# mathworks/turtle_kv

Measured on AMD Instinct MI355X. Metric: filter-build Mkeys/s (device-resident), 16B keys @10 bits/key; bit-exact, higher is better.
Workload: dtype u64; 1 GPU; Bloom @10 bits/key: 100000000 x 16B keys per GPU, 16384-key leaves (6104 filters on rank 0); keys_per_gpu=100000000, total_keys=100000000, key_bytes=16, leaf_keys=16384, bits_per_key=10, filter=bloom-blocked512, parallelism=leaf-sharded x1

## Files before the change

### turtle_kv_amd/_build.py

```python
from __future__ import annotations

import fcntl
import hashlib
import os
import subprocess

HERE = os.path.dirname(os.path.abspath(__file__))
ROOT = os.path.dirname(HERE)
LIB = os.path.join(HERE, "libtkv_amq.so")
SOURCES = [os.path.join(HERE, "csrc", "tkv_amq_kernels.hip"),
           os.path.join(HERE, "csrc", "tkv_amq_open_scan.hip"),
           os.path.join(HERE, "csrc", "tkv_amq_find.hip"),
           os.path.join(HERE, "csrc", "tkv_amq_walk.hip"),
           os.path.join(HERE, "csrc", "tkv_amq_stage.cpp")]
DEPS = SOURCES + [os.path.join(HERE, "csrc", "tkv_amq_device.h"),
                  os.path.join(HERE, "csrc", "tkv_amq_verify.h"),
                  os.path.join(ROOT, "include", "tkv_amq.h")]
HIPCC = os.environ.get("HIPCC", "/opt/rocm/bin/hipcc")
FLAGS = ["-O3", "--offload-arch=gfx950", "-std=c++17", "-shared", "-fPIC",
         "-Wall", "-Wno-unused-function", "-I" + os.path.join(ROOT, "include")]


STAMP = LIB + ".src"
LOCK = LIB + ".lock"


def source_digest() -> str:
    h = hashlib.sha256(" ".join([HIPCC, *FLAGS]).encode())
    for d in DEPS:
        with open(d, "rb") as f:
            h.update(f.read())
    return h.hexdigest()


def stale() -> bool:
    if not (os.path.exists(LIB) and os.path.exists(STAMP)):
        return True
    with open(STAMP) as f:
        return f.read().strip() != source_digest()


def build(force: bool = False) -> str:
    if not force and not stale():
        return LIB
    with open(LOCK, "a") as lk:
        fcntl.flock(lk, fcntl.LOCK_EX)
        try:
            if force or stale():
# ... 18 lines not shown
```

### turtle_kv_amd/csrc/tkv_amq_kernels.hip

```cpp
#include <hip/hip_runtime.h>

#include <algorithm>
#include <mutex>
#include <type_traits>
#include <vector>

#include <math.h>
#include <stdint.h>
#include <string.h>
#include <stdlib.h>

#include "tkv_amq.h"
#include "tkv_amq_device.h"

#if defined(TKV_DIAG_RING) && !defined(TKV_AMQ_EXPERIMENT_BUILD)
#error "TKV_DIAG_RING is a diagnostic: build it only as an experiment library (-DTKV_AMQ_EXPERIMENT_BUILD)"
#endif

namespace tkv {

struct BloomSeeds {
  uint64_t seed[kMaxBloomHashes];
  uint64_t rhinit16[kMaxBloomHashes];
  uint64_t seed_p5[kMaxBloomHashes];
};

constexpr BloomSeeds make_bloom_seeds()
{
  BloomSeeds t{};
  for (uint32_t i = 0; i < kMaxBloomHashes; ++i) {
    t.seed[i] = bloom_seed(i);
    t.rhinit16[i] = xxh16_rhinit(t.seed[i]);
    t.seed_p5[i] = t.seed[i] + kP5;
  }
  return t;
}

__constant__ BloomSeeds c_bloom = make_bloom_seeds();

enum KeyMode : int { kKey16 = 0, kKeyFixed = 1, kKeyVar = 2, kKey24 = 3, kKeyLoc = 4 };

typedef uint32_t u32x4_t __attribute__((ext_vector_type(4)));

__device__ inline uint4 load_nt16(const void* p)
{
  const u32x4_t v = __builtin_nontemporal_load(static_cast<const u32x4_t*>(p));
// ... 94 lines not shown
TKV_INLINE auto with_bloom_key_at(const uint8_t* keys, const uint64_t* offs, uint32_t stride, uint64_t i, F&& f)
{
  uint32_t len;
  const uint8_t* p = key_at<MODE>(keys, offs, stride, i, len);
  if (len < 32) return f(BloomShort(p, len));
  return f(BloomLong{p, len});
}

__device__ inline void lds_barrier()
{
  asm volatile("s_waitcnt lgkmcnt(0)\n\ts_barrier" ::: "memory");
}

__device__ inline void lds_set_bit(uint32_t* blk, uint32_t bit)
{
  uint32_t word;
  asm("v_bfe_u32 %0, %1, 5, 4" : "=v"(word) : "v"(bit));
  atomicOr(blk + word, 1u << (bit & 31));
}

TKV_INLINE void global_set_bit(uint32_t* blk, uint32_t bit)
{
  bit &= kBloomBitMask;
  atomicOr(blk + (bit >> 5), 1u << (bit & 31));
}

typedef __attribute__((address_space(3))) uint32_t lds_u32_t;
__device__ inline uint32_t lds_addr(const void* p)
{
  return (uint32_t)reinterpret_cast<uintptr_t>(p);
}
TKV_INLINE uint32_t* lds_ptr(uint32_t a) { return (uint32_t*)reinterpret_cast<lds_u32_t*>((uintptr_t)a); }

template <int K, bool kMask = false, typename H>
TKV_INLINE void bloom_insert(uint32_t* s_bits, uint32_t nb, uint32_t k, const H& x, uint32_t first = 0)
{
  const uint64_t h0 = x.h0();
  uint32_t block = (uint32_t)bloom_block(h0, nb);
  asm("" : "+v"(block));
  uint32_t* blk = lds_ptr((block << 6) + (lds_addr(s_bits) - (first << 6)));
  lds_set_bit(blk, (uint32_t)h0);
  bloom_ladder<K>(x, k, [&](uint32_t, uint32_t b) { lds_set_bit(blk, kMask ? b & kBloomBitMask : b); });
}

template <int K, int MODE>
__device__ inline void bloom_insert_any(uint32_t* s_bits, uint32_t nb, uint32_t k,
                                        const uint8_t* p, uint32_t len)
{
  if (len < 32) bloom_insert<K>(s_bits, nb, k, BloomShort(p, len));
  else bloom_insert<0, true>(s_bits, nb, k, BloomLong{p, len});
}

__device__ inline void write_bloom_header(uint8_t* payload, const tkv_amq_segment& sg, int part)
{
  uint64_t w0, w1;
  const uint64_t nb = sg.n_blocks;
  switch (part) {
    case 0: w0 = kBloomMagic; w1 = 512ull * nb; break;
    case 1: w0 = sg.src_page_id; w1 = 0; break;
    case 2: w0 = 8ull * nb; w1 = nb | ((uint64_t)sg.hash_count << 32) | (2ull << 48); break;
    default: w0 = sg.n_keys; w1 = 0; break;
  }
  ulonglong2 v;
  v.x = w0;
  v.y = w1;
  reinterpret_cast<ulonglong2*>(payload)[part] = v;
}

constexpr uint64_t kLayoutVqf = 0x746c69665f667176ull;
constexpr uint64_t kLayoutBloom = 0x746c666d6f6f6c62ull;

__device__ inline void write_page_header(uint8_t* out, const tkv_amq_segment& sg, uint64_t layout,
                                         uint32_t part)
{
  if (!(sg.page_flags & TKV_AMQ_PAGE_IMAGE)) return;
  uint8_t* page = out + sg.out_offset - kPackedPageHeaderBytes;
  const uint32_t size = 1u << ((sg.page_flags >> 8) & 31u);
  uint4 v = {0, 0, 0, 0};
  if (part == 1) {
    v.x = (uint32_t)layout;
    v.y = (uint32_t)(layout >> 32);
    v.w = (uint32_t)kPackedPageHeaderBytes + sg.payload_bytes;
  } else if (part == 2) {
// ... 7 lines not shown
TKV_INLINE uint64_t sgpr_addr(const uint8_t* base)
{
  uint64_t a = reinterpret_cast<uint64_t>(base);
  asm("" : "+s"(a));
  return a;
}

template <typename T>
TKV_INLINE T load_sbase(uint64_t sbase, uint32_t lane_off, uint32_t imm = 0)
{
  return *reinterpret_cast<const __attribute__((address_space(1))) T*>(sbase + lane_off + imm);
}

template <int K, uint32_t NT = 256>
__device__ inline void bloom_keys16_lds(const uint4* __restrict__ kp, uint32_t n, uint32_t nb,
                                        uint32_t k, uint32_t* s_bits)
{
  const uint32_t tid = threadIdx.x;
  constexpr int U = 4;
  constexpr uint32_t C = NT * U;
  const uint8_t* cb = reinterpret_cast<const uint8_t*>(kp);
  uint32_t lane_off = tid * 16;
  uint32_t base = 0;
  for (; n - base >= C; base += C, cb += C * 16) {
    asm volatile("" : "+v"(lane_off));
    uint4 kv[U];
#pragma unroll
    for (int u = 0; u < U; ++u) {
      const u32x4_t v = load_sbase<u32x4_t>(sgpr_addr(cb + u * NT * 16), lane_off);
      kv[u] = uint4{v.x, v.y, v.z, v.w};
    }
#pragma unroll
    for (int u = 0; u < U; ++u) {
      bloom_insert<K>(s_bits, nb, k, Bloom16(kv[u]));
      __builtin_amdgcn_sched_barrier(0);
    }
  }
  if (base < n) {
    uint4 kv[U];
#pragma unroll
    for (int u = 0; u < U; ++u) {
      const uint32_t i = base + u * NT + tid;
      if (i < n) kv[u] = kp[i];
    }
#pragma unroll
    for (int u = 0; u < U; ++u) {
      const uint32_t i = base + u * NT + tid;
      if (i < n) bloom_insert<K>(s_bits, nb, k, Bloom16(kv[u]));
    }
  }
}

template <int K, int L, uint32_t NT>
__device__ inline void bloom_keysL_lds(const uint64_t* __restrict__ kp, uint32_t n, uint32_t nb,
                                       uint32_t k, uint32_t* s_bits)
{
  constexpr int N = L / 8;
  const uint32_t tid = threadIdx.x;
  constexpr int U = 2;
  constexpr uint32_t C = NT * U;
  const uint8_t* cb = reinterpret_cast<const uint8_t*>(kp);
  uint32_t lane_off = tid * L;
  uint32_t base = 0;
  for (; n - base >= C; base += C, cb += C * L) {
    asm volatile("" : "+v"(lane_off));
    uint64_t lanes[U][N];
#pragma unroll
    for (int u = 0; u < U; ++u) {
      const uint64_t sb = sgpr_addr(cb + u * NT * L);
#pragma unroll
      for (int w = 0; w < N; ++w) lanes[u][w] = load_sbase<uint64_t>(sb, lane_off, w * 8);
    }
#pragma unroll
    for (int u = 0; u < U; ++u) {
      bloom_insert<K>(s_bits, nb, k, BloomFixed<L>(lanes[u]));
      __builtin_amdgcn_sched_barrier(0);
    }
  }
  if (base < n) {
    uint64_t lanes[U][N];
#pragma unroll
    for (int u = 0; u < U; ++u) {
      const uint32_t i = min(base + u * NT + tid, n - 1);
#pragma unroll
      for (int w = 0; w < N; ++w) lanes[u][w] = kp[(uint64_t)i * N + w];
    }
#pragma unroll
    for (int u = 0; u < U; ++u) {
      if (base + u * NT + tid < n) {
        bloom_insert<K>(s_bits, nb, k, BloomFixed<L>(lanes[u]));
      }
    }
  }
}

template <int MODE, uint32_t NT>
__device__ inline void bloom_leaf_image(const uint8_t* __restrict__ keys,
                                        const uint64_t* __restrict__ offs, uint32_t stride,
                                        const tkv_amq_segment& sg, uint32_t kb, uint32_t ke,
                                        uint32_t* s_bits)
{
  const uint32_t n = ke - kb, nb = sg.n_blocks, k = sg.hash_count;
  if constexpr (MODE == kKey16) {
    const uint4* kp = reinterpret_cast<const uint4*>(keys) + sg.key_begin + kb;
    if (k == 7) bloom_keys16_lds<7, NT>(kp, n, nb, k, s_bits);
    else if (k == 8) bloom_keys16_lds<8, NT>(kp, n, nb, k, s_bits);
    else bloom_keys16_lds<0, NT>(kp, n, nb, k, s_bits);
  } else if constexpr (MODE == kKey24) {
    const uint64_t* kp = reinterpret_cast<const uint64_t*>(keys) + 3 * (sg.key_begin + kb);
    if (n != 0) {
      if (k == 7) bloom_keysL_lds<7, 24, NT>(kp, n, nb, k, s_bits);
      else if (k == 8) bloom_keysL_lds<8, 24, NT>(kp, n, nb, k, s_bits);
      else bloom_keysL_lds<0, 24, NT>(kp, n, nb, k, s_bits);
    }
  } else {
    for (uint32_t i = kb + threadIdx.x; i < ke; i += NT) {
      uint32_t len;
      const uint8_t* p = key_at<MODE>(keys, offs, stride, sg.key_begin + i, len);
      if (k == 7) bloom_insert_any<7, MODE>(s_bits, nb, k, p, len);
      else if (k == 8) bloom_insert_any<8, MODE>(s_bits, nb, k, p, len);
      else bloom_insert_any<0, MODE>(s_bits, nb, k, p, len);
    }
  }
// ... 74 lines not shown
  const bool sh = len < 32;
  const uint32_t n8 = len >> 3, nb = len & 3;
  uint64_t l[3];
#pragma unroll
  for (uint32_t j = 0; j < 3; ++j) l[j] = ld64_unaligned(sh && j < n8 ? p + 8 * j : safe);
  const uint8_t* q = p + 8 * n8;
  const uint32_t t4 = ld32_unaligned(sh && (len & 4) ? q : safe);
  q += len & 4;
  const uint32_t c0 = *(sh && nb > 0 ? q : safe), c1 = *(sh && nb > 1 ? q + 1 : safe),
                 c2 = *(sh && nb > 2 ? q + 2 : safe);
  const uint32_t tb = c0 | c1 << 8 | c2 << 16;
  const uint32_t tlo = (len & 4) ? t4 : tb;
  w.a = u32x4_b{lo32(l[0]), hi32(l[0]), lo32(l[1]), hi32(l[1])};
  w.b = u32x4_b{lo32(l[2]), hi32(l[2]), tlo, tb};
  if (n8 == 0) { w.a.x = tlo; w.a.y = tb; }
  else if (n8 == 1) { w.a.z = tlo; w.a.w = tb; }
  else if (n8 == 2) { w.b.x = tlo; w.b.y = tb; }
  w.d = 0;
}

struct VarKey {
  KeyWin w;
  uint32_t len;
  const uint8_t* p;
};

template <int K>
__device__ inline void var_key_insert(uint32_t* s_bits, uint32_t nb, uint32_t k, const VarKey& v)
{
  if (v.len < 32) {
    uint64_t l[3];
    uint32_t t4, tb;
    key_win_parts(v.w, v.len, l, t4, tb);
    bloom_insert<K>(s_bits, nb, k, BloomShort(v.len, l, t4, tb));
  } else {
    bloom_insert_any<K, kKeyVar>(s_bits, nb, k, v.p, v.len);
  }
}

template <uint32_t NT, int K>
__device__ void bloom_var_sorted_image(const uint8_t* __restrict__ keys, const uint64_t* __restrict__ offs,
                                       const tkv_amq_segment& sg, uint32_t kb, uint32_t ke,
                                       uint32_t* s_bits, uint32_t* s_aux, uint64_t key_end)
{
  constexpr uint32_t C = kVarChunk<NT>, U = C / NT;
  uint32_t* bins = s_aux;
  uint32_t* start = s_aux + kVarBins;
  uint2* kl = reinterpret_cast<uint2*>(s_aux + 2 * kVarBins);
  const uint32_t tid = threadIdx.x, nb = sg.n_blocks, k = sg.hash_count;
  const uint64_t* o = offs + sg.key_begin;
  const uint8_t* safe = reinterpret_cast<const uint8_t*>(offs);
  for (uint32_t c0 = kb; c0 < ke; c0 += C) {
    const uint32_t cn = min(C, ke - c0);
    const uint64_t base = o[c0];
    if (tid < kVarBins) bins[tid] = 0;
    __syncthreads();
    uint32_t bin[U], rank[U], rel[U], len[U];
#pragma unroll
    for (uint32_t u = 0; u < U; ++u) {
      const uint32_t j = u * NT + tid;
      const uint32_t i = c0 + min(j, cn - 1);
      const uint64_t b = o[i];
      const uint64_t l = o[i + 1] - b;
      rel[u] = (uint32_t)(b - base);
      len[u] = (uint32_t)l;
      bin[u] = l < 32 ? (uint32_t)l : 32u;
      rank[u] = j < cn ? atomicAdd(bins + bin[u], 1u) : 0u;
// ... 15 lines not shown
      const uint32_t j = u * NT + tid;
      if (j < cn) kl[start[bin[u]] + rank[u]] = make_uint2(rel[u], len[u]);
    }
    __syncthreads();
    const uint8_t* kbase = keys + base;
    const VarRsrc vr = var_rsrc(keys, base, o[c0 + cn], key_end);
    VarKey A, B;
    auto load = [&](uint32_t q, VarKey& v) {
      const uint2 e = kl[min(q, cn - 1)];
      if (vr.nrec) key_win_load(vr, e.x, v.w);
      else key_win_load_clamped(kbase + e.x, e.y, safe, v.w);
      v.len = e.y;
      v.p = kbase + e.x;
    };
    load(tid, A);
    for (uint32_t q = tid; q < cn; q += 2 * NT) {
      load(q + NT, B);
      var_key_insert<K>(s_bits, nb, k, A);
      if (q + NT >= cn) break;
      load(q + 2 * NT, A);
      var_key_insert<K>(s_bits, nb, k, B);
    }
    __syncthreads();
  }
}

template <int MODE, uint32_t NT>
__global__ __launch_bounds__(NT) void bloom_build_lds(const uint8_t* __restrict__ keys,
                                                       const uint64_t* __restrict__ offs,
                                                       uint32_t stride,
                                                       const tkv_amq_segment* __restrict__ segs,
                                                       uint8_t* __restrict__ out, uint32_t var_sort)
{
  extern __shared__ uint32_t s_lds[];
  const bool sorted = MODE == kKeyVar && var_sort;
  uint32_t* s_bits = s_lds + (sorted ? kVarAuxWords<NT> : 0u);
  const tkv_amq_segment sg = segs[blockIdx.x];
  const uint32_t n = sg.n_keys, nb = sg.n_blocks, k = sg.hash_count;
  if (k == 0) return;
  const uint32_t tid = threadIdx.x;
  const uint32_t nwords = nb * 16;

  for (uint32_t w = tid; w < nwords; w += NT) s_bits[w] = 0;
  __syncthreads();
  if constexpr (MODE == kKeyVar) {
    if (sorted) {
      const tkv_amq_segment& last = segs[gridDim.x - 1];
      const uint64_t key_end = offs[last.key_begin + last.n_keys];
      if (k == 7) bloom_var_sorted_image<NT, 7>(keys, offs, sg, 0, n, s_bits, s_lds, key_end);
      else if (k == 8) bloom_var_sorted_image<NT, 8>(keys, offs, sg, 0, n, s_bits, s_lds, key_end);
      else bloom_var_sorted_image<NT, 0>(keys, offs, sg, 0, n, s_bits, s_lds, key_end);
    } else {
      bloom_leaf_image<MODE, NT>(keys, offs, stride, sg, 0, n, s_bits);
    }
  } else {
    bloom_leaf_image<MODE, NT>(keys, offs, stride, sg, 0, n, s_bits);
  }
  __syncthreads();

  uint8_t* payload = out + sg.out_offset;
  if (tid < 4) write_bloom_header(payload, sg, tid);
  else if (tid < 8) write_page_header(out, sg, kLayoutBloom, tid - 4);
  uint4* dst = reinterpret_cast<uint4*>(payload + kBloomHeader);
  const uint4* src = reinterpret_cast<const uint4*>(s_bits);
  for (uint32_t q = tid; q < nb * 4; q += NT) dst[q] = src[q];
}

constexpr uint32_t kSplitThreads = 512;
constexpr uint32_t kSplitMaxParts = 16;
constexpr uint32_t kMergeThreads = 256;

template <int MODE>
__global__ __launch_bounds__(kSplitThreads) void bloom_build_split(
    const uint8_t* __restrict__ keys, const uint64_t* __restrict__ offs, uint32_t stride,
    const tkv_amq_segment* __restrict__ segs, uint32_t parts, uint8_t* __restrict__ ws,
    uint64_t img_stride)
{
  constexpr uint32_t NT = kSplitThreads;
  extern __shared__ uint32_t s_bits[];
  const uint32_t seg = blockIdx.x / parts, part = blockIdx.x - seg * parts;
  const tkv_amq_segment sg = segs[seg];
  const uint32_t n = sg.n_keys, nb = sg.n_blocks;
  if (sg.hash_count == 0) return;
  const uint32_t tid = threadIdx.x;
  for (uint32_t w = tid; w < nb * 16; w += NT) s_bits[w] = 0;
  __syncthreads();
  const uint32_t chunk = (n + parts - 1) / parts;
  const uint32_t kb = min(n, part * chunk), ke = min(n, kb + chunk);
  bloom_leaf_image<MODE, NT>(keys, offs, stride, sg, kb, ke, s_bits);
  __syncthreads();
  const uint4* img = reinterpret_cast<const uint4*>(s_bits);
  uint4* dst = reinterpret_cast<uint4*>(ws + (uint64_t)blockIdx.x * img_stride);
  for (uint32_t q = tid; q < nb * 4; q += NT) dst[q] = img[q];
}

__global__ __launch_bounds__(kMergeThreads) void bloom_split_merge(
    const tkv_amq_segment* __restrict__ segs, uint32_t parts, uint32_t chunks,
    const uint8_t* __restrict__ ws, uint64_t img_stride, uint8_t* __restrict__ out)
{
  const uint32_t seg = blockIdx.x / chunks, c = blockIdx.x - seg * chunks;
  const tkv_amq_segment sg = segs[seg];
  if (sg.hash_count == 0) return;
  const uint32_t tid = threadIdx.x, nq = sg.n_blocks * 4;
  uint8_t* payload = out + sg.out_offset;
  if (c == 0 && tid < 4) write_bloom_header(payload, sg, tid);
  else if (c == 0 && tid < 8) write_page_header(out, sg, kLayoutBloom, tid - 4);
  const uint32_t q = c * kMergeThreads + tid;
  if (q >= nq) return;
  const uint8_t* base = ws + (uint64_t)seg * parts * img_stride + 16ull * q;
  uint4 o[kSplitMaxParts];
#pragma unroll
  for (uint32_t p = 0; p < kSplitMaxParts; ++p)
    o[p] = p < parts ? load_nt16(base + (uint64_t)p * img_stride) : make_uint4(0, 0, 0, 0);
  uint4 v = o[0];
#pragma unroll
  for (uint32_t p = 1; p < kSplitMaxParts; ++p) {
    v.x |= o[p].x;
    v.y |= o[p].y;
    v.z |= o[p].z;
    v.w |= o[p].w;
  }
  reinterpret_cast<uint4*>(payload + kBloomHeader)[q] = v;
}

constexpr uint32_t kWinThreads = 1024;
constexpr uint32_t kWinMaxWindows = 16;
// ... 43 lines not shown
                                    const WinKey<MODE>& kb, WinItem<MODE>& it)
{
  uint64_t h0;
  if constexpr (MODE == kKey16) {
    const Bloom16 x(kb.v);
    h0 = x.h0();
    it.d[0] = lo32(x.rk1);
    it.d[1] = hi32(x.rk1);
    it.d[2] = lo32(x.k2);
    it.d[3] = hi32(x.k2);
  } else if constexpr (MODE == kKey24) {
    const BloomFixed<24> x(kb.w);
    h0 = x.h0();
    it.d[0] = lo32(x.rk0);
    it.d[1] = hi32(x.rk0);
    it.d[2] = lo32(x.k[0]);
    it.d[3] = hi32(x.k[0]);
    it.d[4] = lo32(x.k[1]);
    it.d[5] = hi32(x.k[1]);
  } else {
    h0 = bloom_h0_at<MODE>(keys, offs, stride, sg.key_begin + i);
    it.d[0] = i;
  }
  it.d[WinItem<MODE>::N - 1] = ((uint32_t)h0 & kBloomBitMask) << 12;
  return (uint32_t)bloom_block(h0, sg.n_blocks);
}

template <int MODE, int K>
__device__ inline void win_insert(const uint8_t* __restrict__ keys, const uint64_t* __restrict__ offs,
                                  uint32_t stride, const tkv_amq_segment& sg, uint32_t k,
                                  const WinItem<MODE>& it, uint32_t* s_bits)
{
  const uint32_t loc = it.d[WinItem<MODE>::N - 1];
  uint32_t* blk = s_bits + 16 * (loc & 0xfffu);
  lds_set_bit(blk, loc >> 12);
  if constexpr (MODE == kKey16) {
    Bloom16 x;
    x.rk1 = mk64(it.d[0], it.d[1]);
    x.k2 = mk64(it.d[2], it.d[3]);
    if constexpr (K != 0) {
#pragma unroll
      for (uint32_t j = 1; j < (uint32_t)K; ++j) lds_set_bit(blk, x.bit(j));
    } else {
      for (uint32_t j = 1; j < k; ++j) lds_set_bit(blk, x.bit(j));
    }
  } else if constexpr (MODE == kKey24) {
    BloomFixed<24> x;
    x.rk0 = mk64(it.d[0], it.d[1]);
    x.k[0] = mk64(it.d[2], it.d[3]);
    x.k[1] = mk64(it.d[4], it.d[5]);
    if constexpr (K != 0) {
#pragma unroll
      for (uint32_t j = 1; j < (uint32_t)K; ++j) lds_set_bit(blk, x.bit(j));
    } else {
      for (uint32_t j = 1; j < k; ++j) lds_set_bit(blk, x.bit(j));
    }
  } else {
    uint32_t len;
    const uint8_t* p = key_at<MODE>(keys, offs, stride, sg.key_begin + it.d[0], len);
    const uint32_t kk = K != 0 ? (uint32_t)K : k;
    if (len < 32) {
      const BloomShort x(p, len);
      for (uint32_t j = 1; j < kk; ++j) lds_set_bit(blk, x.bit(j));
    } else {
      const BloomLong x{p, len};
      for (uint32_t j = 1; j < kk; ++j) lds_set_bit(blk, x.bit(j));
    }
  }
}

__device__ inline uint32_t mbcnt64(uint64_t m)
{
  return __builtin_amdgcn_mbcnt_hi((uint32_t)(m >> 32), __builtin_amdgcn_mbcnt_lo((uint32_t)m, 0u));
}

template <int MODE, int K>
__device__ void bloom_window_keys(const uint8_t* __restrict__ keys, const uint64_t* __restrict__ offs,
                                  uint32_t stride, const tkv_amq_segment& sg, uint32_t wb, uint32_t wn,
                                  uint32_t kb, uint32_t ke, uint32_t* s_bits)
{
  constexpr int N = WinItem<MODE>::N;
  constexpr uint32_t NW = kWinThreads / 64;
  const uint32_t lane = threadIdx.x & 63u, wave = threadIdx.x >> 6;
  const uint32_t k = sg.hash_count;
  if (ke <= kb) return;
  WinItem<MODE> pend;
#pragma unroll
  for (int d = 0; d < N; ++d) pend.d[d] = 0;
  uint32_t c = 0;
  auto step = [&](uint32_t base, const WinKey<MODE>& cur) {
    const uint32_t i = base + lane;
    WinItem<MODE> it;
    const uint32_t lb = win_hash<MODE>(keys, offs, stride, sg, min(i, ke - 1), cur, it) - wb;
    const bool in = i < ke && lb < wn;
    it.d[N - 1] |= lb & 0xfffu;
    const uint64_t mask = __ballot(in);
    const uint32_t m = (uint32_t)__popcll(mask);
    if (m == 0) return;
    const uint32_t rank = mbcnt64(in ? mask : ~mask) + (in ? 0u : m);
// ... 7 lines not shown
      for (int d = 0; d < N; ++d) full.d[d] = lane < c ? pend.d[d] : pm.d[d];
      win_insert<MODE, K>(keys, offs, stride, sg, k, full, s_bits);
      pend = pm;
      c = c + m - 64;
    } else {
#pragma unroll
      for (int d = 0; d < N; ++d) pend.d[d] = lane < c ? pend.d[d] : pm.d[d];
      c += m;
    }
  };
  constexpr bool kPre = MODE == kKey16 || MODE == kKey24;
  auto load = [&](uint32_t base, WinKey<MODE>& kv) {
    if constexpr (kPre) win_load<MODE>(keys, sg.key_begin + min(base + lane, ke - 1), kv);
  };
  WinKey<MODE> A{}, B{};
  uint32_t base = kb + wave * 64;
  load(base, A);
  for (; base < ke; base += 2 * NW * 64) {
    load(base + NW * 64, B);
    step(base, A);
    if (base + NW * 64 >= ke) break;
    load(base + 2 * NW * 64, A);
    step(base + NW * 64, B);
  }
  if (lane < c) win_insert<MODE, K>(keys, offs, stride, sg, k, pend, s_bits);
}

template <int MODE>
__global__ __launch_bounds__(kWinThreads) void bloom_build_window(
    const uint8_t* __restrict__ keys, const uint64_t* __restrict__ offs, uint32_t stride,
    const tkv_amq_segment* __restrict__ segs, uint32_t n_win, uint32_t win_blocks, uint32_t parts,
    uint8_t* __restrict__ ws, uint64_t img_stride, uint8_t* __restrict__ out)
{
  extern __shared__ uint32_t s_bits[];
  const uint32_t per_seg = n_win * parts;
  const uint32_t seg = blockIdx.x / per_seg, r = blockIdx.x - seg * per_seg;
  const uint32_t w = r / parts, part = r - w * parts;
  const tkv_amq_segment sg = segs[seg];
  const uint32_t nb = sg.n_blocks, n = sg.n_keys, k = sg.hash_count;
  const uint32_t wb = w * win_blocks;
  if (k == 0 || wb >= nb) return;
  const uint32_t wn = min(win_blocks, nb - wb);
  const uint32_t tid = threadIdx.x;
  for (uint32_t q = tid; q < wn * 16; q += kWinThreads) s_bits[q] = 0;
  __syncthreads();
  const uint32_t chunk = (n + parts - 1) / parts;
  const uint32_t kb = min(n, part * chunk), ke = min(n, kb + chunk);
  if (nb <= win_blocks) {
    bloom_leaf_image<MODE, kWinThreads>(keys, offs, stride, sg, kb, ke, s_bits);
  } else if (k == 7) {
    bloom_window_keys<MODE, 7>(keys, offs, stride, sg, wb, wn, kb, ke, s_bits);
  } else if (k == 8) {
    bloom_window_keys<MODE, 8>(keys, offs, stride, sg, wb, wn, kb, ke, s_bits);
  } else {
    bloom_window_keys<MODE, 0>(keys, offs, stride, sg, wb, wn, kb, ke, s_bits);
  }
  __syncthreads();
  uint8_t* dst8;
  if (parts == 1) {
    uint8_t* payload = out + sg.out_offset;
    if (w == 0 && tid < 4) write_bloom_header(payload, sg, tid);
    else if (w == 0 && tid < 8) write_page_header(out, sg, kLayoutBloom, tid - 4);
    dst8 = payload + kBloomHeader + 64ull * wb;
  } else {
    dst8 = ws + (uint64_t)(seg * parts + part) * img_stride + 64ull * wb;
  }
  uint4* dst = reinterpret_cast<uint4*>(dst8);
  const uint4* src = reinterpret_cast<const uint4*>(s_bits);
  for (uint32_t q = tid; q < wn * 4; q += kWinThreads) dst[q] = src[q];
}

__global__ __launch_bounds__(256) void bloom_global_init(const tkv_amq_segment* __restrict__ segs,
                                                         uint8_t* __restrict__ out)
{
  const tkv_amq_segment sg = segs[blockIdx.x];
  if (sg.hash_count == 0) return;
  uint8_t* payload = out + sg.out_offset;
  const uint32_t tid = threadIdx.x;
  if (tid < 4) write_bloom_header(payload, sg, tid);
  else if (tid < 8) write_page_header(out, sg, kLayoutBloom, tid - 4);
  uint4* dst = reinterpret_cast<uint4*>(payload + kBloomHeader);
  const uint4 z = {0, 0, 0, 0};
  for (uint64_t q = tid; q < 4ull * sg.n_blocks; q += 256) dst[q] = z;
}

__device__ inline uint32_t find_segment(const tkv_amq_segment* segs, uint32_t n_segs,
                                        uint64_t key)
{
  uint32_t lo = 0, hi = n_segs;
  while (hi - lo > 1) {
    const uint32_t mid = (lo + hi) >> 1;
    if (segs[mid].key_begin <= key) lo = mid;
    else hi = mid;
  }
  return lo;
}

template <int MODE>
__global__ __launch_bounds__(256) void bloom_global_set(const uint8_t* __restrict__ keys,
                                                        const uint64_t* __restrict__ offs,
                                                        uint32_t stride,
                                                        const tkv_amq_segment* __restrict__ segs,
// ... 3596 lines not shown

template <typename Fn>
inline void with_flag(bool on, Fn&& fn)
{
  if (on) fn(std::true_type{});
  else fn(std::false_type{});
}

constexpr int kMaxDevices = 64;
template <typename Fn>
inline void once_per_device(std::once_flag (&flags)[kMaxDevices], Fn&& fn)
{
  int dev = 0;
  if (hipGetDevice(&dev) != hipSuccess || dev < 0 || dev >= kMaxDevices) {
    fn();
    return;
  }
  std::call_once(flags[dev], fn);
}

template <auto K, typename... A>
inline void launch_lds_cap(uint32_t cap, dim3 grid, dim3 block, size_t lds, hipStream_t s, A&&... a)
{
  static std::once_flag flags[kMaxDevices];
  once_per_device(flags, [cap] {
    (void)hipFuncSetAttribute(reinterpret_cast<const void*>(K), hipFuncAttributeMaxDynamicSharedMemorySize, (int)cap);
  });
  hipLaunchKernelGGL(K, grid, block, lds, s, std::forward<A>(a)...);
}

constexpr uint32_t kBloomLdsBudget = 64 * 1024;
constexpr uint32_t kBloomLeafLdsBudget = 160 * 1024;
constexpr uint32_t kBloomWideLds = 32 * 1024;
constexpr uint32_t kBloomSpreadSegs = 64;
constexpr uint32_t kBloomSplitSegs = 256;
constexpr uint32_t kSplitTargetWgs = 1024;
constexpr uint32_t kSplitMinKeys = 1024;
constexpr uint32_t kBloomWideSegs = 2048;

inline uint32_t bloom_split_parts(uint32_t n_segs, uint64_t n_keys, uint64_t max_blocks)
{
  if (n_segs == 0 || n_segs >= kBloomSplitSegs || 64 * max_blocks > kBloomLeafLdsBudget) return 1;
  uint64_t p = (kSplitTargetWgs + n_segs - 1) / n_segs;
  const uint64_t per_leaf = n_keys / n_segs;
  const uint64_t by_keys = per_leaf / kSplitMinKeys;
  if (p > by_keys) p = by_keys;
  if (p > kSplitMaxParts) p = kSplitMaxParts;
  return p < 2 ? 1u : (uint32_t)p;
}

inline uint64_t bloom_split_ws_bytes(uint32_t n_segs, uint32_t parts, uint64_t max_blocks)
{
  return parts < 2 ? 0 : (uint64_t)n_segs * parts * 64 * max_blocks;
}

constexpr uint32_t kWinMonoMax = 1;
constexpr uint32_t kChipCUs = 256;

inline uint32_t bloom_window_count(uint64_t max_blocks)
{
  return (uint32_t)div_up(64 * max_blocks, kBloomLeafLdsBudget);
}

inline uint32_t bloom_window_blocks(uint64_t max_blocks)
{
  return (uint32_t)div_up(max_blocks, bloom_window_count(max_blocks));
// ... 657 lines not shown
  r.kind = TKV_AMQ_LEAF_BATCH;
  if (!batch_tiled(g.n_blocks, fixed)) return r;
  r.kind = TKV_AMQ_LEAF_NONE;
  if (g.bits_per_key == 0) return r;
  if (fixed && multi_leaf(g.n_keys, g.n_blocks)) {
    r.pg = multi_geom(g.n_keys, g.n_blocks, wg_items);
    r.kind = TKV_AMQ_LEAF_MULTI;
    if (rest_bytes > kSplitImgBytes && align256(r.pg.bytes) <= rest_bytes - kSplitImgBytes) return r;
  }
  r.plan = bloom_leaf_route(g, bmode, true, rest_bytes);
  r.kind = r.plan.route == BloomRoute::TiledKeys      ? TKV_AMQ_LEAF_TILED_KEYS
           : r.plan.route == BloomRoute::TiledRecords ? TKV_AMQ_LEAF_TILED_RECORDS
                                                      : TKV_AMQ_LEAF_ATOMICS;
  return r;
}

struct BuildArgs {
  const uint8_t* keys; const uint64_t* offs; uint32_t stride; uint64_t n_keys;
  const tkv_amq_segment* d_segs; uint32_t n_segs, max_blocks; uint8_t* d_out;
  void* d_ws; uint64_t ws_bytes; hipStream_t s; int mode, bmode;
};

inline void launch_split_merge(const BuildArgs& b, uint32_t parts)
{
  const uint32_t chunks = (uint32_t)div_up(4ull * b.max_blocks, kMergeThreads);
  hipLaunchKernelGGL(bloom_split_merge, dim3(b.n_segs * chunks), dim3(kMergeThreads), 0, b.s, b.d_segs, parts, chunks,
                     static_cast<uint8_t*>(b.d_ws), 64ull * b.max_blocks, b.d_out);
}

inline void launch_bloom_split(const BuildArgs& b, const BloomPlan& p)
{
  with_build_key_mode(b.bmode, [&](auto M) {
    launch_lds_cap<&bloom_build_split<decltype(M)::value>>(
        kBloomLeafLdsBudget, dim3(b.n_segs * p.parts), dim3(kSplitThreads), 64ull * b.max_blocks, b.s, b.keys, b.offs,
        b.stride, b.d_segs, p.parts, static_cast<uint8_t*>(b.d_ws), 64ull * b.max_blocks);
  });
  launch_split_merge(b, p.parts);
}

inline void launch_bloom_window(const BuildArgs& b, const BloomPlan& p)
{
  with_build_key_mode(b.bmode, [&](auto M) {
    launch_lds_cap<&bloom_build_window<decltype(M)::value>>(
        kBloomLeafLdsBudget, dim3(b.n_segs * p.windows * p.parts), dim3(kWinThreads), 64ull * p.window_blocks, b.s,
        b.keys, b.offs, b.stride, b.d_segs, p.windows, p.window_blocks, p.parts, static_cast<uint8_t*>(b.d_ws),
        64ull * b.max_blocks, b.d_out);
  });
  if (p.parts > 1) launch_split_merge(b, p.parts);
}

inline void launch_bloom_atomics(hipStream_t s, int mode, const uint8_t* keys, const uint64_t* offs, uint32_t stride,
                                 const tkv_amq_segment* d_segs, uint32_t n_segs, uint64_t key0, uint64_t key_end,
                                 uint8_t* d_out)
{
  hipLaunchKernelGGL(bloom_global_init, dim3(n_segs), dim3(256), 0, s, d_segs, d_out);
  const uint32_t g2 = (uint32_t)std::min<uint64_t>(div_up(key_end - key0, 256), 8192);
  if (g2)
    with_key_mode(mode, [&](auto M) {
      hipLaunchKernelGGL(bloom_global_set<decltype(M)::value>, dim3(g2), dim3(256), 0, s, keys, offs, stride, d_segs,
                         n_segs, key_end, d_out, key0);
    });
}

enum class VqfDecide : uint32_t { BigU8 = TKV_AMQ_ROUTE_VQF_BIG_U8, BigGlobal, RingPlace, RingPlace2, Ring, Decide };
enum class VqfPlace : uint32_t { None = TKV_AMQ_PLACE_NONE, Fused512, Fused256, Scatter };
static_assert((uint32_t)VqfDecide::Decide == TKV_AMQ_ROUTE_VQF_DECIDE && (uint32_t)VqfPlace::Scatter == TKV_AMQ_PLACE_SCATTER, "");

struct VqfPlan {
  VqfDecide decide;
  VqfPlace place;
  bool located;
  size_t lds;
  size_t rl;
  uint32_t cw, tbl;
  int flags;
  uint32_t place_parts, place_span;
  uint32_t key_wgs;
// ... 275 lines not shown

int tkv_amq_build(int kind, const uint8_t* keys, const uint64_t* offs, uint32_t stride,
                  uint64_t n_keys, const tkv_amq_segment* d_segs, uint32_t n_segs,
                  uint32_t max_blocks, uint8_t* d_out, void* d_ws, uint64_t ws_bytes, void* stream)
{
  return build_batch(kind, keys, offs, stride, n_keys, d_segs, n_segs, max_blocks, d_out, d_ws, ws_bytes,
                     stream, n_keys);
}

static int build_batch(int kind, const uint8_t* keys, const uint64_t* offs, uint32_t stride,
                       uint64_t n_keys, const tkv_amq_segment* d_segs, uint32_t n_segs,
                       uint32_t max_blocks, uint8_t* d_out, void* d_ws, uint64_t ws_bytes, void* stream,
                       uint64_t sizing_keys)
{
  if (tkv_amq_device_count() == 0) return TKV_AMQ_UNAVAILABLE;
  if (n_segs == 0) return TKV_AMQ_OK;
  if (!d_segs || !d_out || (n_keys && !keys) || (!offs && stride == 0))
    return TKV_AMQ_INVALID_ARGUMENT;
  const hipStream_t s = as_stream(stream);
  const int mode = key_mode(offs, stride);
  if (mode == kKey16 && (reinterpret_cast<uintptr_t>(keys) & 15)) return TKV_AMQ_INVALID_ARGUMENT;
  const BuildArgs b{keys, offs, stride, n_keys, d_segs, n_segs, max_blocks, d_out, d_ws, ws_bytes, s, mode,
                    build_key_mode(keys, offs, stride)};

  if (kind == TKV_AMQ_BLOOM) {
    if (max_blocks == 0) return TKV_AMQ_OK;
    const BloomPlan p = bloom_route(n_segs, sizing_keys, max_blocks, b.bmode, bloom_k_of(sizing_keys, max_blocks),
                                    d_ws != nullptr, ws_bytes);
    uint8_t* ws = static_cast<uint8_t*>(d_ws);
    switch (p.route) {
      case BloomRoute::Split: launch_bloom_split(b, p); break;
      case BloomRoute::Window: launch_bloom_window(b, p); break;
      case BloomRoute::Lds:
        if (p.threads == 1024) launch_bloom_lds<1024>(b.bmode, n_segs, 64ull * max_blocks, s, keys, offs, stride, d_segs, d_out);
        else launch_bloom_lds<256>(b.bmode, n_segs, 64ull * max_blocks, s, keys, offs, stride, d_segs, d_out);
        break;
      case BloomRoute::TiledKeys:
        launch_mono(p.mono, s, keys, b.bmode == kKey24 ? 24u : 16u, (uint32_t)sizing_keys, d_segs, ws, d_out);
        break;
      case BloomRoute::TiledRecords:
        launch_any(p.any, bloom_k_of(sizing_keys, max_blocks), s, keys, mode == kKeyVar ? offs : nullptr, stride,
                   (uint32_t)sizing_keys, d_segs, ws, d_out);
        break;
      case BloomRoute::Atomics: launch_bloom_atomics(s, mode, keys, offs, stride, d_segs, n_segs, 0, n_keys, d_out); break;
    }
    return hipGetLastError() == hipSuccess ? TKV_AMQ_OK : TKV_AMQ_INTERNAL;
  }

  if (kind != TKV_AMQ_VQF) return TKV_AMQ_INVALID_ARGUMENT;
  if (max_blocks == 0) {
    if (d_ws && ws_bytes >= 64 && hipMemsetAsync(static_cast<uint8_t*>(d_ws) + 4, 0, 4, s) != hipSuccess)
      return TKV_AMQ_INTERNAL;
    return TKV_AMQ_OK;
  }
  if (max_blocks > kVqfMaxBlocks) return TKV_AMQ_RESOURCE_EXHAUSTED;
  if (!d_ws) return TKV_AMQ_INVALID_ARGUMENT;
  if (ws_bytes < vqf_temp_offset(n_segs) + kVqfTempStride * (uint64_t)max_blocks + 8 * n_keys)
    return TKV_AMQ_INVALID_ARGUMENT;
  const VqfPlan p = vqf_route(n_segs, max_blocks, b.bmode, n_keys);
  const dim3 dg(n_segs), wave(64);
  with_build_key_mode(b.bmode, [&](auto M) {
    constexpr int MODE = decltype(M)::value;
    switch (p.decide) {
      case VqfDecide::BigU8:
        launch_lds_cap<&vqf_decide_big<MODE, kCntU8>>(kVqfLdsCap, dg, wave, p.lds, s, keys, offs, stride, d_segs, d_ws,
                                                      ws_bytes, n_segs);
        break;
      case VqfDecide::BigGlobal:
// ... 691 lines not shown
```

Before: 146,000 Mkeys/s.

## Interleave Bloom block words across LDS regions to spread atomic bank traffic

Replaces the contiguous 64-byte-per-block LDS filter image with a strided layout. Eight blocks share a 512-byte region, and word w of each block sits at a 32-byte stride. Random block and bit choices should then land on more distinct LDS banks during the atomicOr inserts. Zeroing and the copy-out loops are rewritten to de-interleave back to the canonical layout, and LDS sizes are rounded up to whole regions. The cost is slightly more address arithmetic (two v_bfi per insert) and a gathered read pattern on write-out.

```diff
diff --git a/turtle_kv_amd/_build.py b/turtle_kv_amd/_build.py
--- a/turtle_kv_amd/_build.py
+++ b/turtle_kv_amd/_build.py
@@ -14,6 +14,7 @@
            os.path.join(HERE, "csrc", "tkv_amq_walk.hip"),
            os.path.join(HERE, "csrc", "tkv_amq_stage.cpp")]
 DEPS = SOURCES + [os.path.join(HERE, "csrc", "tkv_amq_device.h"),
+                  os.path.join(HERE, "csrc", "tkv_amq_lds_stride.h"),
                   os.path.join(HERE, "csrc", "tkv_amq_verify.h"),
                   os.path.join(ROOT, "include", "tkv_amq.h")]
 HIPCC = os.environ.get("HIPCC", "/opt/rocm/bin/hipcc")
diff --git a/turtle_kv_amd/csrc/tkv_amq_kernels.hip b/turtle_kv_amd/csrc/tkv_amq_kernels.hip
--- a/turtle_kv_amd/csrc/tkv_amq_kernels.hip
+++ b/turtle_kv_amd/csrc/tkv_amq_kernels.hip
@@ -12,6 +12,7 @@
 
 #include "tkv_amq.h"
 #include "tkv_amq_device.h"
+#include "tkv_amq_lds_stride.h"
 
 #if defined(TKV_DIAG_RING) && !defined(TKV_AMQ_EXPERIMENT_BUILD)
 #error "TKV_DIAG_RING is a diagnostic: build it only as an experiment library (-DTKV_AMQ_EXPERIMENT_BUILD)"
@@ -172,23 +173,69 @@
 }
 TKV_INLINE uint32_t* lds_ptr(uint32_t a) { return (uint32_t*)reinterpret_cast<lds_u32_t*>((uintptr_t)a); }
 
-template <int K, bool kMask = false, typename H>
+TKV_INLINE uint32_t lds_stride_key4(uint32_t image_base, uint32_t b4)
+{
+  const uint32_t t = (b4 << 4) + image_base;
+  uint32_t x;
+  asm("v_bfi_b32 %0, %1, %2, %3" : "=v"(x) : "n"(kStrideSlotMask), "v"(b4), "v"(t));
+  return x;
+}
+TKV_INLINE uint32_t lds_stride_key(uint32_t image_base, uint32_t local_block)
+{
+  return lds_stride_key4(image_base, local_block << 2);
+}
+
+TKV_INLINE void lds_set_bit_strided(uint32_t x, uint32_t bit)
+{
+  uint32_t a;
+  asm("v_bfi_b32 %0, %1, %2, %3" : "=v"(a) : "s"(kStrideWordMask), "v"(bit), "v"(x));
+  atomicOr(lds_ptr(a), 1u << (bit & 31));
+}
+
+template <uint32_t NT>
+TKV_INLINE void lds_stride_zero(uint32_t* s_bits, uint32_t nb)
+{
+  const uint32_t nq = lds_stride_words(nb) / 4;
+  uint4* img = reinterpret_cast<uint4*>(s_bits);
+  for (uint32_t q = threadIdx.x; q < nq; q += NT) img[q] = make_uint4(0, 0, 0, 0);
+}
+
+template <uint32_t NT>
+TKV_INLINE void lds_stride_write_out(uint32_t* s_bits, uint32_t nb, uint4* __restrict__ dst)
+{
+  static_assert(NT % (4 * kStrideRegionBlocks) == 0, "a lane's quads must keep their slot and row");
+  const uint32_t tid = threadIdx.x, nq = nb * 4;
+  uint32_t a = lds_addr(s_bits) + lds_stride_quad(tid);
+  for (uint32_t q = tid; q < nq; q += NT, a += NT * 16) {
+    const uint32_t* p = lds_ptr(a);
+    constexpr uint32_t W = kStrideWordBytes / 4;
+    dst[q] = make_uint4(p[0], p[W], p[2 * W], p[3 * W]);
+  }
+}
+
+template <int K, bool kMask = false, bool kStride = false, typename H>
 TKV_INLINE void bloom_insert(uint32_t* s_bits, uint32_t nb, uint32_t k, const H& x, uint32_t first = 0)
 {
   const uint64_t h0 = x.h0();
-  uint32_t block = (uint32_t)bloom_block(h0, nb);
+  uint32_t block = (uint32_t)bloom_block(h0, kStride ? nb * 4u : nb);
   asm("" : "+v"(block));
-  uint32_t* blk = lds_ptr((block << 6) + (lds_addr(s_bits) - (first << 6)));
-  lds_set_bit(blk, (uint32_t)h0);
-  bloom_ladder<K>(x, k, [&](uint32_t, uint32_t b) { lds_set_bit(blk, kMask ? b & kBloomBitMask : b); });
+  if constexpr (kStride) {
+    const uint32_t sx = lds_stride_key4(lds_addr(s_bits), block - first * 4u);
+    lds_set_bit_strided(sx, (uint32_t)h0);
+    bloom_ladder<K>(x, k, [&](uint32_t, uint32_t b) { lds_set_bit_strided(sx, b); });
+  } else {
+    uint32_t* blk = lds_ptr((block << 6) + (lds_addr(s_bits) - (first << 6)));
+    lds_set_bit(blk, (uint32_t)h0);
+    bloom_ladder<K>(x, k, [&](uint32_t, uint32_t b) { lds_set_bit(blk, kMask ? b & kBloomBitMask : b); });
+  }
 }
 
 template <int K, int MODE>
 __device__ inline void bloom_insert_any(uint32_t* s_bits, uint32_t nb, uint32_t k,
                                         const uint8_t* p, uint32_t len)
 {
-  if (len < 32) bloom_insert<K>(s_bits, nb, k, BloomShort(p, len));
-  else bloom_insert<0, true>(s_bits, nb, k, BloomLong{p, len});
+  if (len < 32) bloom_insert<K, false, true>(s_bits, nb, k, BloomShort(p, len));
+  else bloom_insert<0, false, true>(s_bits, nb, k, BloomLong{p, len});
 }
 
 __device__ inline void write_bloom_header(uint8_t* payload, const tkv_amq_segment& sg, int part)
@@ -262,7 +309,7 @@
     }
 #pragma unroll
     for (int u = 0; u < U; ++u) {
-      bloom_insert<K>(s_bits, nb, k, Bloom16(kv[u]));
+      bloom_insert<K, false, true>(s_bits, nb, k, Bloom16(kv[u]));
       __builtin_amdgcn_sched_barrier(0);
     }
   }
@@ -276,7 +323,7 @@
 #pragma unroll
     for (int u = 0; u < U; ++u) {
       const uint32_t i = base + u * NT + tid;
-      if (i < n) bloom_insert<K>(s_bits, nb, k, Bloom16(kv[u]));
+      if (i < n) bloom_insert<K, false, true>(s_bits, nb, k, Bloom16(kv[u]));
     }
   }
 }
@@ -303,7 +350,7 @@
     }
 #pragma unroll
     for (int u = 0; u < U; ++u) {
-      bloom_insert<K>(s_bits, nb, k, BloomFixed<L>(lanes[u]));
+      bloom_insert<K, false, true>(s_bits, nb, k, BloomFixed<L>(lanes[u]));
       __builtin_amdgcn_sched_barrier(0);
     }
   }
@@ -318,7 +365,7 @@
 #pragma unroll
     for (int u = 0; u < U; ++u) {
       if (base + u * NT + tid < n) {
-        bloom_insert<K>(s_bits, nb, k, BloomFixed<L>(lanes[u]));
+        bloom_insert<K, false, true>(s_bits, nb, k, BloomFixed<L>(lanes[u]));
       }
     }
   }
@@ -459,7 +506,7 @@
     uint64_t l[3];
     uint32_t t4, tb;
     key_win_parts(v.w, v.len, l, t4, tb);
-    bloom_insert<K>(s_bits, nb, k, BloomShort(v.len, l, t4, tb));
+    bloom_insert<K, false, true>(s_bits, nb, k, BloomShort(v.len, l, t4, tb));
   } else {
     bloom_insert_any<K, kKeyVar>(s_bits, nb, k, v.p, v.len);
   }
@@ -541,16 +588,16 @@
                                                        const tkv_amq_segment* __restrict__ segs,
                                                        uint8_t* __restrict__ out, uint32_t var_sort)
 {
-  extern __shared__ uint32_t s_lds[];
+  extern __shared__ __attribute__((aligned(kStrideRegionBytes))) uint32_t s_lds[];
+  static_assert(4 * kVarAuxWords<NT> % kStrideRegionBytes == 0, "the image behind the scratch must stay region-aligned");
   const bool sorted = MODE == kKeyVar && var_sort;
   uint32_t* s_bits = s_lds + (sorted ? kVarAuxWords<NT> : 0u);
   const tkv_amq_segment sg = segs[blockIdx.x];
   const uint32_t n = sg.n_keys, nb = sg.n_blocks, k = sg.hash_count;
   if (k == 0) return;
   const uint32_t tid = threadIdx.x;
-  const uint32_t nwords = nb * 16;
-
-  for (uint32_t w = tid; w < nwords; w += NT) s_bits[w] = 0;
+
+  lds_stride_zero<NT>(s_bits, nb);
   __syncthreads();
   if constexpr (MODE == kKeyVar) {
     if (sorted) {
@@ -570,9 +617,7 @@
   uint8_t* payload = out + sg.out_offset;
   if (tid < 4) write_bloom_header(payload, sg, tid);
   else if (tid < 8) write_page_header(out, sg, kLayoutBloom, tid - 4);
-  uint4* dst = reinterpret_cast<uint4*>(payload + kBloomHeader);
-  const uint4* src = reinterpret_cast<const uint4*>(s_bits);
-  for (uint32_t q = tid; q < nb * 4; q += NT) dst[q] = src[q];
+  lds_stride_write_out<NT>(s_bits, nb, reinterpret_cast<uint4*>(payload + kBloomHeader));
 }
 
 constexpr uint32_t kSplitThreads = 512;
@@ -586,21 +631,18 @@
     uint64_t img_stride)
 {
   constexpr uint32_t NT = kSplitThreads;
-  extern __shared__ uint32_t s_bits[];
+  extern __shared__ __attribute__((aligned(kStrideRegionBytes))) uint32_t s_bits[];
   const uint32_t seg = blockIdx.x / parts, part = blockIdx.x - seg * parts;
   const tkv_amq_segment sg = segs[seg];
   const uint32_t n = sg.n_keys, nb = sg.n_blocks;
   if (sg.hash_count == 0) return;
-  const uint32_t tid = threadIdx.x;
-  for (uint32_t w = tid; w < nb * 16; w += NT) s_bits[w] = 0;
+  lds_stride_zero<NT>(s_bits, nb);
   __syncthreads();
   const uint32_t chunk = (n + parts - 1) / parts;
   const uint32_t kb = min(n, part * chunk), ke = min(n, kb + chunk);
   bloom_leaf_image<MODE, NT>(keys, offs, stride, sg, kb, ke, s_bits);
   __syncthreads();
-  const uint4* img = reinterpret_cast<const uint4*>(s_bits);
-  uint4* dst = reinterpret_cast<uint4*>(ws + (uint64_t)blockIdx.x * img_stride);
-  for (uint32_t q = tid; q < nb * 4; q += NT) dst[q] = img[q];
+  lds_stride_write_out<NT>(s_bits, nb, reinterpret_cast<uint4*>(ws + (uint64_t)blockIdx.x * img_stride));
 }
 
 __global__ __launch_bounds__(kMergeThreads) void bloom_split_merge(
@@ -710,17 +752,17 @@
                                   const WinItem<MODE>& it, uint32_t* s_bits)
 {
   const uint32_t loc = it.d[WinItem<MODE>::N - 1];
-  uint32_t* blk = s_bits + 16 * (loc & 0xfffu);
-  lds_set_bit(blk, loc >> 12);
+  const uint32_t blk = lds_stride_key(lds_addr(s_bits), loc & 0xfffu);
+  lds_set_bit_strided(blk, loc >> 12);
   if constexpr (MODE == kKey16) {
     Bloom16 x;
     x.rk1 = mk64(it.d[0], it.d[1]);
     x.k2 = mk64(it.d[2], it.d[3]);
     if constexpr (K != 0) {
 #pragma unroll
-      for (uint32_t j = 1; j < (uint32_t)K; ++j) lds_set_bit(blk, x.bit(j));
+      for (uint32_t j = 1; j < (uint32_t)K; ++j) lds_set_bit_strided(blk, x.bit(j));
     } else {
-      for (uint32_t j = 1; j < k; ++j) lds_set_bit(blk, x.bit(j));
+      for (uint32_t j = 1; j < k; ++j) lds_set_bit_strided(blk, x.bit(j));
     }
   } else if constexpr (MODE == kKey24) {
     BloomFixed<24> x;
@@ -729,9 +771,9 @@
     x.k[1] = mk64(it.d[4], it.d[5]);
     if constexpr (K != 0) {
 #pragma unroll
-      for (uint32_t j = 1; j < (uint32_t)K; ++j) lds_set_bit(blk, x.bit(j));
+      for (uint32_t j = 1; j < (uint32_t)K; ++j) lds_set_bit_strided(blk, x.bit(j));
     } else {
-      for (uint32_t j = 1; j < k; ++j) lds_set_bit(blk, x.bit(j));
+      for (uint32_t j = 1; j < k; ++j) lds_set_bit_strided(blk, x.bit(j));
     }
   } else {
     uint32_t len;
@@ -739,10 +781,10 @@
     const uint32_t kk = K != 0 ? (uint32_t)K : k;
     if (len < 32) {
       const BloomShort x(p, len);
-      for (uint32_t j = 1; j < kk; ++j) lds_set_bit(blk, x.bit(j));
+      for (uint32_t j = 1; j < kk; ++j) lds_set_bit_strided(blk, x.bit(j));
     } else {
       const BloomLong x{p, len};
-      for (uint32_t j = 1; j < kk; ++j) lds_set_bit(blk, x.bit(j));
+      for (uint32_t j = 1; j < kk; ++j) lds_set_bit_strided(blk, x.bit(j));
     }
   }
 }
@@ -816,7 +858,7 @@
     const tkv_amq_segment* __restrict__ segs, uint32_t n_win, uint32_t win_blocks, uint32_t parts,
     uint8_t* __restrict__ ws, uint64_t img_stride, uint8_t* __restrict__ out)
 {
-  extern __shared__ uint32_t s_bits[];
+  extern __shared__ __attribute__((aligned(kStrideRegionBytes))) uint32_t s_bits[];
   const uint32_t per_seg = n_win * parts;
   const uint32_t seg = blockIdx.x / per_seg, r = blockIdx.x - seg * per_seg;
   const uint32_t w = r / parts, part = r - w * parts;
@@ -826,7 +868,7 @@
   if (k == 0 || wb >= nb) return;
   const uint32_t wn = min(win_blocks, nb - wb);
   const uint32_t tid = threadIdx.x;
-  for (uint32_t q = tid; q < wn * 16; q += kWinThreads) s_bits[q] = 0;
+  lds_stride_zero<kWinThreads>(s_bits, wn);
   __syncthreads();
   const uint32_t chunk = (n + parts - 1) / parts;
   const uint32_t kb = min(n, part * chunk), ke = min(n, kb + chunk);
@@ -849,9 +891,7 @@
   } else {
     dst8 = ws + (uint64_t)(seg * parts + part) * img_stride + 64ull * wb;
   }
-  uint4* dst = reinterpret_cast<uint4*>(dst8);
-  const uint4* src = reinterpret_cast<const uint4*>(s_bits);
-  for (uint32_t q = tid; q < wn * 4; q += kWinThreads) dst[q] = src[q];
+  lds_stride_write_out<kWinThreads>(s_bits, wn, reinterpret_cast<uint4*>(dst8));
 }
 
 __global__ __launch_bounds__(256) void bloom_global_init(const tkv_amq_segment* __restrict__ segs,
@@ -4514,6 +4554,10 @@
 constexpr uint32_t kBloomLdsBudget = 64 * 1024;
 constexpr uint32_t kBloomLeafLdsBudget = 160 * 1024;
 constexpr uint32_t kBloomWideLds = 32 * 1024;
+inline size_t bloom_image_lds(uint64_t blocks) { return (size_t)lds_stride_bytes64(blocks); }
+static_assert(kBloomLeafLdsBudget % kStrideRegionBytes == 0 && kBloomWideLds % kStrideRegionBytes == 0 &&
+                  kBloomLdsBudget % kStrideRegionBytes == 0,
+              "a rounded-up image must fit where the canonical one does");
 constexpr uint32_t kBloomSpreadSegs = 64;
 constexpr uint32_t kBloomSplitSegs = 256;
 constexpr uint32_t kSplitTargetWgs = 1024;
@@ -5237,7 +5281,7 @@
 {
   with_build_key_mode(b.bmode, [&](auto M) {
     launch_lds_cap<&bloom_build_split<decltype(M)::value>>(
-        kBloomLeafLdsBudget, dim3(b.n_segs * p.parts), dim3(kSplitThreads), 64ull * b.max_blocks, b.s, b.keys, b.offs,
+        kBloomLeafLdsBudget, dim3(b.n_segs * p.parts), dim3(kSplitThreads), bloom_image_lds(b.max_blocks), b.s, b.keys, b.offs,
         b.stride, b.d_segs, p.parts, static_cast<uint8_t*>(b.d_ws), 64ull * b.max_blocks);
   });
   launch_split_merge(b, p.parts);
@@ -5247,7 +5291,7 @@
 {
   with_build_key_mode(b.bmode, [&](auto M) {
     launch_lds_cap<&bloom_build_window<decltype(M)::value>>(
-        kBloomLeafLdsBudget, dim3(b.n_segs * p.windows * p.parts), dim3(kWinThreads), 64ull * p.window_blocks, b.s,
+        kBloomLeafLdsBudget, dim3(b.n_segs * p.windows * p.parts), dim3(kWinThreads), bloom_image_lds(p.window_blocks), b.s,
         b.keys, b.offs, b.stride, b.d_segs, p.windows, p.window_blocks, p.parts, static_cast<uint8_t*>(b.d_ws),
         64ull * b.max_blocks, b.d_out);
   });
@@ -5589,8 +5633,8 @@
       case BloomRoute::Split: launch_bloom_split(b, p); break;
       case BloomRoute::Window: launch_bloom_window(b, p); break;
       case BloomRoute::Lds:
-        if (p.threads == 1024) launch_bloom_lds<1024>(b.bmode, n_segs, 64ull * max_blocks, s, keys, offs, stride, d_segs, d_out);
-        else launch_bloom_lds<256>(b.bmode, n_segs, 64ull * max_blocks, s, keys, offs, stride, d_segs, d_out);
+        if (p.threads == 1024) launch_bloom_lds<1024>(b.bmode, n_segs, bloom_image_lds(max_blocks), s, keys, offs, stride, d_segs, d_out);
+        else launch_bloom_lds<256>(b.bmode, n_segs, bloom_image_lds(max_blocks), s, keys, offs, stride, d_segs, d_out);
         break;
       case BloomRoute::TiledKeys:
         launch_mono(p.mono, s, keys, b.bmode == kKey24 ? 24u : 16u, (uint32_t)sizing_keys, d_segs, ws, d_out);
diff --git a/turtle_kv_amd/csrc/tkv_amq_lds_stride.h b/turtle_kv_amd/csrc/tkv_amq_lds_stride.h
--- /dev/null
+++ b/turtle_kv_amd/csrc/tkv_amq_lds_stride.h
@@ -0,0 +1,35 @@
+#pragma once
+
+#include <stdint.h>
+
+#if defined(__HIPCC__) || defined(__CUDACC__)
+#define TKV_STRIDE_FN __host__ __device__ constexpr
+#else
+#define TKV_STRIDE_FN constexpr
+#endif
+
+namespace tkv {
+
+constexpr uint32_t kStrideRegionBlocks = 8;
+constexpr uint32_t kStrideRegionBytes = 512;
+constexpr uint32_t kStrideWordBytes = 32;
+constexpr uint32_t kStrideWordMask = 0x1e0;
+constexpr uint32_t kStrideSlotMask = 0x1c;
+
+TKV_STRIDE_FN uint32_t lds_stride_bytes(uint32_t nb) { return ((nb + 7u) >> 3) * kStrideRegionBytes; }
+TKV_STRIDE_FN uint32_t lds_stride_words(uint32_t nb) { return lds_stride_bytes(nb) / 4u; }
+TKV_STRIDE_FN uint64_t lds_stride_bytes64(uint64_t nb) { return ((nb + 7u) >> 3) * kStrideRegionBytes; }
+
+TKV_STRIDE_FN uint32_t lds_stride_block(uint32_t b) { return ((b >> 3) << 9) | ((b & 7u) << 2); }
+TKV_STRIDE_FN uint32_t lds_stride_addr(uint32_t b, uint32_t w) { return lds_stride_block(b) | (w << 5); }
+TKV_STRIDE_FN uint32_t lds_stride_bit_addr(uint32_t b, uint32_t bit)
+{
+  return (lds_stride_block(b) & ~kStrideWordMask) | (bit & kStrideWordMask);
+}
+
+TKV_STRIDE_FN uint32_t lds_stride_block_of(uint32_t a) { return ((a >> 9) << 3) | ((a >> 2) & 7u); }
+TKV_STRIDE_FN uint32_t lds_stride_word_of(uint32_t a) { return (a >> 5) & 15u; }
+
+TKV_STRIDE_FN uint32_t lds_stride_quad(uint32_t q) { return lds_stride_addr(q >> 2, 4u * (q & 3u)); }
+
+}
```

Measured after the change: 148,500 Mkeys/s, median of 6. 1.7% higher.
